# google-research/nerf-from-image

Hardware: AMD Instinct MI355X
Metric: rendered rays/sec (128x128, 64+64 samples) (higher is better)
Workload: dtype f32 (decoder MLP operands split-fp16 hi+lo, 22 bits; strict fp32: config.value_mlp_exact_fp32)

## Files before the change

include/nfi_hip.h:

```cpp
#ifndef NFI_HIP_H
#define NFI_HIP_H

#include <stddef.h>
#include <stdint.h>

#ifdef __cplusplus
extern "C" {
#endif

typedef void* nfi_stream_t;

typedef enum nfi_status {
  NFI_OK = 0,
  NFI_ERR_INVALID_ARGUMENT = -1,
  NFI_ERR_UNSUPPORTED = -2,
  NFI_ERR_WORKSPACE_TOO_SMALL = -3,
  NFI_ERR_LAUNCH = -4
} nfi_status;

enum { NFI_PLANE_CHANNELS = 32, NFI_HIDDEN = 64, NFI_MAX_ATTENTION = 14, NFI_MAX_SAMPLES = 128 };
enum { NFI_MAX_SAMPLES_SINGLE_PASS = 512 };

enum { NFI_TEXEL_F32 = 0, NFI_TEXEL_BF16 = 1, NFI_TEXEL_F16 = 2 };
enum { NFI_TEXELS_PLANAR = 0, NFI_TEXELS_INTERLEAVED = 1 };
// ... 67 lines not shown
  int n_attention;
  const float* attention_values;
  int use_sdf;
  const float* beta;
  const float* alpha;
  float scene_range;
  float* sigma;
  float* rgb;
  float* sdf;
  float* semantics;
  uint8_t* outside;
  const float* ray_features;
  int samples_per_ray;
  int texel_layout;
  int mlp_precision;
} nfi_field_args;
int nfi_field_query_fwd(const nfi_field_args* a, nfi_stream_t stream);
const char* nfi_field_kernel_name(const nfi_field_args* a);

int nfi_bbox_overlay(const float* points, int64_t n_points, float scene_range, float threshold, const float* sigma_in,
                     float* sigma_out, nfi_stream_t stream);

typedef struct nfi_weights_args {
  int64_t n_rays;
  int n_samples;
  const float* sigma;
  const float* ray_directions;
  const float* depth;
  float* weights;
} nfi_weights_args;
int nfi_ray_weights(const nfi_weights_args* a, nfi_stream_t stream);

typedef struct nfi_sample_pdf_args {
  int64_t n_rays;
  int n_bins;
  int n_samples;
  const float* bins;
  const float* weights;
  const float* u;
  int64_t u_row_stride;
  float* samples;
  int64_t* inds;
  float* cdf;
} nfi_sample_pdf_args;
int nfi_sample_pdf(const nfi_sample_pdf_args* a, nfi_stream_t stream);

typedef struct nfi_resample_args {
  int64_t n_rays;
  int n_samples;
  const float* sigma;
  const float* ray_directions;
  const float* depth;
  const float* u;
  int64_t u_row_stride;
  float* fine_depth;
  float* weights;
  float* smooth;
  float* cdf;
  int64_t* inds;
} nfi_resample_args;
int nfi_resample(const nfi_resample_args* a, nfi_stream_t stream);

typedef struct nfi_composite_args {
  int64_t n_rays;
  int n_a;
  int n_b;
  const float* ray_directions;
  const float* depth_a; const float* sigma_a; const float* rgb_a;
  const float* depth_b; const float* sigma_b; const float* rgb_b;
  int n_extra;
  const float* extra_a;
  const float* extra_b;
  int white_background;
  float* rgb_map;
  float* depth_map;
  float* mask;
  float* extra_map;
  float* weights;
  float* depth_sorted;
  int64_t* perm;
} nfi_composite_args;
int nfi_composite_fwd(const nfi_composite_args* a, nfi_stream_t stream);

typedef struct nfi_composite_bwd_args {
  int64_t n_rays;
  int n_a; int n_b;
  const float* ray_directions;
  const float* depth_a; const float* sigma_a; const float* rgb_a;
  const float* depth_b; const float* sigma_b; const float* rgb_b;
  int n_extra; const float* extra_a; const float* extra_b;
  int white_background;
  const float* g_rgb_map;
  const float* g_mask;
  const float* g_extra_map;
  float* g_sigma_a; float* g_rgb_a;
  float* g_sigma_b; float* g_rgb_b;
  float* g_extra_a; float* g_extra_b;
  float* g_ray_directions;
  int list_row_stride;
} nfi_composite_bwd_args;
int nfi_composite_bwd(const nfi_composite_bwd_args* a, nfi_stream_t stream);
int nfi_points_bwd(const float* g_points, const float* depth, int64_t n_rays, int n_samples,
                   float* g_ray_origins, float* g_ray_directions, nfi_stream_t stream);
int nfi_raygen_bwd(const nfi_raygen_args* a, const float* g_ray_origins, const float* g_ray_directions,
                   float* g_cam2world, float* g_focal, nfi_stream_t stream);
int nfi_raygen_bwd_ordered(const nfi_raygen_args* a, const float* g_ray_origins, const float* g_ray_directions,
                           float* g_cam2world, float* g_focal, nfi_stream_t stream);

typedef struct nfi_field_bwd_args {
  int n_scenes;
  int64_t points_per_scene;
  const float* points;
  const void* texels; int plane_res; int texel_dtype;
  const float* decoder_image;
  const float* w1; const float* w2;
  int n_attention; const float* attention_values;
  int use_sdf; const float* beta; const float* alpha;
  float scene_range;
  const float* g_sigma; const float* g_rgb; const float* g_sdf; const float* g_semantics;
  float* g_texels; float* g_points;
  float* g_w1; float* g_b1; float* g_w2; float* g_b2;
  float* g_attention_values; float* g_beta; float* g_alpha;
  void* workspace; size_t workspace_bytes;
  int points_only; int normalize_g_points;
  const float* ray_features; int samples_per_ray; const float* w3;
  float* g_ray_features; float* g_w3; float* g_b3;
  int scatter_mode;
  int texel_layout;
  int rays_per_row;
} nfi_field_bwd_args;
size_t nfi_field_bwd_workspace_bytes(const nfi_field_bwd_args* a);
size_t nfi_decoder_bwd_image_floats(void);
size_t nfi_decoder_bwd_image_floats_viewdir(void);
int nfi_field_query_bwd(const nfi_field_bwd_args* a, nfi_stream_t stream);
const char* nfi_field_bwd_kernel_name(const nfi_field_bwd_args* a);

typedef struct nfi_sdf_gradient_args {
  int n_scenes;
  int64_t points_per_scene;
  const float* points;
  const float* texels; int plane_res;
  float scene_range;
  const float* w1; const float* b1; const float* w2; const float* b2;
  float* sdf; float* gradient;
  const float* g_sdf; const float* g_gradient;
  float* g_texels; float* g_w1; float* g_b1; float* g_w2; float* g_b2;
  int texel_layout;
} nfi_sdf_gradient_args;
int nfi_sdf_gradient_fwd(const nfi_sdf_gradient_args* a, nfi_stream_t stream);
int nfi_sdf_gradient_bwd(const nfi_sdf_gradient_args* a, nfi_stream_t stream);
size_t nfi_sdf_gradient_bwd_ordered_workspace_bytes(const nfi_sdf_gradient_args* a);
int nfi_sdf_gradient_bwd_ordered(const nfi_sdf_gradient_args* a, void* workspace, size_t workspace_bytes, nfi_stream_t stream);

enum { NFI_TUNING_SCANLINE_ORDER = 4, NFI_TUNING_EXACT_FP32_MLP = 8, NFI_TUNING_SINGLE_WORK_COUNTER = 16 };
typedef struct nfi_render_args {
  int n_scenes, height, width;
  int n_samples;
  int fine_sampling;
  int white_background;
  float scene_range;
  int views_per_scene;
  const float* cam2world; const float* focal; const float* bbox; const float* center;
  const void* texels; int plane_res; int texel_dtype;
  const float* decoder_image; int n_attention; const float* attention_values;
  int use_sdf; const float* beta; const float* alpha;
  const float* noise_coarse;
  const float* noise_fine;
  int64_t noise_fine_row_stride;
  float* rgb;
  float* depth;
  float* mask;
  float* semantics;
  float* ray_origins; float* ray_directions; float* near_plane; float* far_plane; uint8_t* hit;
  float* t_coarse; float* sigma_coarse; float* rgb_coarse;
  float* t_fine; float* sigma_fine; float* rgb_fine;
  float* t_sorted; float* weights; int32_t* perm;
  void* workspace; size_t workspace_bytes;
  int skip_missed_rays;
  void* event_start; void* event_stop;
  int tuning;
  void* profile_cycles;
  const float* ray_features;
  float termination_eps;
  int texel_layout;
  void* clock_probe;
  int row_offset; int full_height;
  float* stash_t; float* stash_sigma; float* stash_rgb;
  int rays_ready;
  float* coords;
  float* normals;
} nfi_render_args;
size_t nfi_render_workspace_bytes(int64_t n_rays);
int nfi_render_fwd(const nfi_render_args* a, nfi_stream_t stream);
const char* nfi_render_kernel_name(const nfi_render_args* a);
int nfi_render_setup(const nfi_render_args* a, nfi_stream_t stream);

typedef struct nfi_pnp_args {
  int n_images; int height; int width;
  const float* coords;
  const float* mask;
  float mask_threshold;
  int n_focal; const float* focal_proposals;
  int refine_iterations;
  void* workspace; size_t workspace_bytes;
  float* world2cam;
  float* focal;
  float* error;
} nfi_pnp_args;
size_t nfi_pnp_workspace_bytes(int n_images, int n_focal);
int nfi_pose_pnp(const nfi_pnp_args* a, nfi_stream_t stream);

typedef struct nfi_torgb_args {
  int n_scenes, in_channels, resolution;
  const float* x; const float* styles; const float* weight; const float* bias; const float* previous_image;
  float* texels;
  const float* g_texels;
  float* g_x; float* g_styles; float* g_weight; float* g_bias; float* g_previous_image;
} nfi_torgb_args;
int nfi_torgb_texels_fwd(const nfi_torgb_args* a, nfi_stream_t stream);
int nfi_torgb_texels_bwd(const nfi_torgb_args* a, nfi_stream_t stream);
size_t nfi_torgb_texels_bwd_ordered_workspace_bytes(const nfi_torgb_args* a);
int nfi_torgb_texels_bwd_ordered(const nfi_torgb_args* a, void* workspace, size_t workspace_bytes, nfi_stream_t stream);

typedef struct nfi_warp_args {
  int n_images, channels, height, width;
  const float* image; float* warped;
  const float* g_warped; float* g_image;
  const float* rot; const float* scale; const float* translation;
  int white_background;
} nfi_warp_args;
int nfi_affine_warp_fwd(const nfi_warp_args* a, nfi_stream_t stream);
int nfi_affine_warp_bwd(const nfi_warp_args* a, nfi_stream_t stream);
int nfi_affine_warp_bwd_ordered(const nfi_warp_args* a, nfi_stream_t stream);

typedef struct nfi_metrics_args {
  int n_images;
  const float* pred; const float* target; int64_t elements_per_image;
  const float* mask_pred; const float* mask_real; int64_t elements_per_mask;
  float* psnr; float* iou; int* out_of_range;
} nfi_metrics_args;
int nfi_image_metrics(const nfi_metrics_args* a, nfi_stream_t stream);

typedef struct nfi_viewdir_mapper_args {
  int64_t n_rays;
  const float* viewdir;
  const float *fc0_w, *fc0_b;
  const float *fc1_w, *norm1_w, *norm1_b;
  const float *fc2_w, *norm2_w, *norm2_b;
  const float *fc3_w, *norm3_w, *norm3_b;
  const float *fc4_w, *norm4_w, *norm4_b;
  const float *fc5_w, *fc5_b, *fc6_w, *fc6_b;
  float* feature;
  const float* g_feature;
  float *g_fc0_w, *g_fc0_b;
  float *g_fc1_w, *g_norm1_w, *g_norm1_b;
  float *g_fc2_w, *g_norm2_w, *g_norm2_b;
  float *g_fc3_w, *g_norm3_w, *g_norm3_b;
  float *g_fc4_w, *g_norm4_w, *g_norm4_b;
  float *g_fc5_w, *g_fc5_b, *g_fc6_w, *g_fc6_b;
  float* g_viewdir;
} nfi_viewdir_mapper_args;
int nfi_viewdir_mapper_fwd(const nfi_viewdir_mapper_args* a, nfi_stream_t stream);
int nfi_viewdir_mapper_bwd(const nfi_viewdir_mapper_args* a, nfi_stream_t stream);

#ifdef __cplusplus
}
#endif
#endif
```

nerf_from_image_amd/csrc/nfi_kernels.hip:

```cpp
#include "nfi_device.hpp"
#include "../../include/nfi_hip.h"
#include "nfi_host.hpp"

#include <algorithm>
#include <cstddef>
#include <cstdio>
#include <cstring>

using namespace nfi;

thread_local char nfi_err_buf[256] = "";
extern "C" const char* nfi_last_error(void) { return nfi_err_buf; }
extern "C" int nfi_version(void) { return 102; }


constexpr int kP2tPixels = 256, kP2tPitch = 288;
template <int TEX>
__global__ __launch_bounds__(256) void planes_to_texels_kernel(const float* __restrict__ planes, void* __restrict__ texels,
                                                               int hw) {
  __shared__ __attribute__((aligned(16))) float tile[kC][kP2tPitch];
  const int img = blockIdx.y;
  const int px0 = blockIdx.x * kP2tPixels;
  const float* src = planes + (size_t)img * kC * hw;
  {
// ... 1068 lines not shown
  const int64_t ray = (int64_t)blockIdx.x * 4 + wave;
  if (ray >= a.n_rays) return;
  WaveSlab& slab = slabs[wave];
  const int S = a.n_samples;
  float sigma[2], t[2], u[2], z[2], w[2], sm[2];
  int ind[2];
#pragma unroll
  for (int j = 0; j < 2; ++j) {
    const int e = j * 64 + lane;
    sigma[j] = e < S ? a.sigma[ray * S + e] : 0.0f;
    t[j] = e < S ? a.depth[ray * S + e] : 0.0f;
    u[j] = e < S ? a.u[ray * a.u_row_stride + e] : 0.0f;
  }
  float dn = norm3(a.ray_directions[ray * 3], a.ray_directions[ray * 3 + 1], a.ray_directions[ray * 3 + 2]);
  float Tc[2];
  resample_ray_wide<2>(slab, sigma, t, S, dn, u, lane, z, w, sm, ind, Tc);
#pragma unroll
  for (int j = 0; j < 2; ++j) {
    const int e = j * 64 + lane;
    if (e < S) {
      a.fine_depth[ray * S + e] = z[j];
      if (a.weights) a.weights[ray * S + e] = w[j];
      if (a.smooth) a.smooth[ray * S + e] = sm[j];
      if (a.inds) a.inds[ray * S + e] = ind[j];
    }
    if (a.cdf && e < S - 1) a.cdf[ray * (S - 1) + e] = slab.cdf[e];
  }
}

extern "C" int nfi_resample(const nfi_resample_args* a, nfi_stream_t stream) {
  REQUIRE(a && a->sigma && a->ray_directions && a->depth && a->u && a->fine_depth, "resample: null pointer");
  REQUIRE(a->n_rays > 0 && a->n_samples >= 4 && a->n_samples <= NFI_MAX_SAMPLES, "resample: n_samples must be in [4,128]");
  const dim3 grid((unsigned)((a->n_rays + 3) / 4));
  if (a->n_samples <= 64) hipLaunchKernelGGL(resample_kernel, grid, dim3(256), 0, (hipStream_t)stream, *a);
  else hipLaunchKernelGGL(resample_wide_kernel, grid, dim3(256), 0, (hipStream_t)stream, *a);
  return check_launch("resample");
}

template <int NS>
__global__ __launch_bounds__(256) void composite_kernel(nfi_composite_args a) {
  __shared__ WaveSlabT<64 * NS> slabs[4];
  const int lane = lane_id();
  const int wave = threadIdx.x >> 6;
  const int64_t ray = (int64_t)blockIdx.x * 4 + wave;
  if (ray >= a.n_rays) return;
  auto& slab = slabs[wave];
  const int na = a.n_a, nb = a.n_b, n = na + nb;
  float dep[NS], sig[NS], cr[NS], cg[NS], cb[NS];
  int eidx[NS];
#pragma unroll
  for (int j = 0; j < NS; ++j) {
    int e = j * 64 + lane;
    dep[j] = sig[j] = cr[j] = cg[j] = cb[j] = 0.0f;
    eidx[j] = e;
    if (e < na) {
      size_t i = (size_t)ray * na + e;
      dep[j] = a.depth_a[i]; sig[j] = a.sigma_a[i];
      cr[j] = a.rgb_a[i * 3]; cg[j] = a.rgb_a[i * 3 + 1]; cb[j] = a.rgb_a[i * 3 + 2];
    } else if (e < n) {
      size_t i = (size_t)ray * nb + (e - na);
      dep[j] = a.depth_b[i]; sig[j] = a.sigma_b[i];
      cr[j] = a.rgb_b[i * 3]; cg[j] = a.rgb_b[i * 3 + 1]; cb[j] = a.rgb_b[i * 3 + 2];
    }
  }
  int rank[NS];
  if (nb > 0) {
    merge_scatter<NS>(slab, dep, sig, cr, cg, cb, eidx, n, rank);
  } else {
#pragma unroll
    for (int j = 0; j < NS; ++j) {
      int e = j * 64 + lane;
      rank[j] = e;
      if (e < n) { slab.srt[0][e] = dep[j]; slab.srt[1][e] = sig[j]; slab.srt[2][e] = cr[j]; slab.srt[3][e] = cg[j]; slab.srt[4][e] = cb[j]; }
    }
    wave_lds_fence();
  }
  float dn = norm3(a.ray_directions[ray * 3], a.ray_directions[ray * 3 + 1], a.ray_directions[ray * 3 + 2]);
  float w[NS];
  CompositeOut o = composite_slab<NS>(slab, n, dn, a.white_background, lane, w);
  if (lane == 0) {
    a.rgb_map[ray * 3] = o.r; a.rgb_map[ray * 3 + 1] = o.g; a.rgb_map[ray * 3 + 2] = o.b;
    a.depth_map[ray] = o.depth;
    a.mask[ray] = o.mask;
  }
#pragma unroll
  for (int j = 0; j < NS; ++j) {
    int e = j * 64 + lane;
    if (e < n) {
      if (a.weights) a.weights[(size_t)ray * n + e] = w[j];
      if (a.depth_sorted) a.depth_sorted[(size_t)ray * n + e] = slab.srt[0][e];
      if (a.perm) a.perm[(size_t)ray * n + rank[j]] = e;
    }
  }
  if (a.n_extra > 0 && a.extra_map) {
    wave_lds_fence();
#pragma unroll
    for (int j = 0; j < NS; ++j) {
      int e = j * 64 + lane;
      if (e < n) slab.cdf[e] = w[j];
    }
    wave_lds_fence();
    float we[NS];
#pragma unroll
    for (int j = 0; j < NS; ++j) { int e = j * 64 + lane; we[j] = e < n ? slab.cdf[rank[j]] : 0.0f; }
    for (int c = 0; c < a.n_extra; ++c) {
      float acc = 0.0f;
#pragma unroll
      for (int j = 0; j < NS; ++j) {
        int e = j * 64 + lane;
        if (e < na) acc += we[j] * a.extra_a[((size_t)ray * na + e) * a.n_extra + c];
        else if (e < n) acc += we[j] * a.extra_b[((size_t)ray * nb + (e - na)) * a.n_extra + c];
      }
      acc = wave_sum(acc);
      if (lane == 0) a.extra_map[ray * a.n_extra + c] = acc;
    }
  }
}

extern "C" int nfi_composite_fwd(const nfi_composite_args* a, nfi_stream_t stream) {
  REQUIRE(a && a->ray_directions && a->depth_a && a->sigma_a && a->rgb_a && a->rgb_map && a->depth_map && a->mask,
          "composite: null pointer");
  REQUIRE(a->n_rays > 0 && a->n_a > 0 && a->n_b >= 0 && a->n_a + a->n_b <= NFI_MAX_SAMPLES_SINGLE_PASS,
          "composite: need 1 <= n_a + n_b <= 512");
  REQUIRE(a->n_b == 0 || (a->n_a <= NFI_MAX_SAMPLES && a->n_b <= NFI_MAX_SAMPLES), "composite: merged lists hold at most 128 samples each");
  REQUIRE(a->n_b == 0 || (a->depth_b && a->sigma_b && a->rgb_b), "composite: list b missing");
  REQUIRE(a->n_extra == 0 || (a->extra_a && (a->n_b == 0 || a->extra_b)), "composite: extra attribute missing");
  const dim3 grid((unsigned)((a->n_rays + 3) / 4));
  if (a->n_a + a->n_b <= 128) hipLaunchKernelGGL(composite_kernel<2>, grid, dim3(256), 0, (hipStream_t)stream, *a);
  else if (a->n_a + a->n_b <= 256) hipLaunchKernelGGL(composite_kernel<4>, grid, dim3(256), 0, (hipStream_t)stream, *a);
  else hipLaunchKernelGGL(composite_kernel<8>, grid, dim3(256), 0, (hipStream_t)stream, *a);
  return check_launch("composite_fwd");
}

#include "nfi_backward_rays.inc"
#include "nfi_regulariser.inc"
#include "nfi_neighbours.inc"
#include "nfi_handoff.inc"
#include "nfi_pnp.inc"
#include "nfi_viewdir_mapper.inc"

struct RenderKernelParams {
  int n_scenes, hw, S;
  int fine, white;
  float scene_range;
  const float* ro; const float* rd; const float* near_raw; const float* far_raw; const uint8_t* hit;
  const uint32_t* reduce;
  uint32_t* counter;
  int width;
  int tile_order;
  int xcd_blocks;
  uint32_t* xcd_counter;
  int xcd_block_shift;
  int fetch_batch;
  const void* texels; int res; int layout;
  const float* image; int A; const float* att;
  int use_sdf; const float* beta; const float* alpha;
  const float* noise_c; const float* noise_f; int64_t noise_f_stride;
  float* rgb; float* depth; float* mask;
  float* near_plane; float* far_plane;
  float* t_coarse; float* sigma_coarse; float* rgb_coarse;
  float* t_fine; float* sigma_fine; float* rgb_fine;
  float* t_sorted; float* weights; int32_t* perm;
  int skip_missed;
  unsigned long long* prof;
  const float* xray;
  float term_eps;
  float* semantics;
  float* coords;
  float* normals;
  unsigned long long* clock_probe;
  FastDiv div_scene_rays, div_bps, div_bw;
  int tap_stride;
  int stash;
};

struct ClockProbe {
  unsigned long long c0 = 0, r0 = 0;
  bool on = false;
  __device__ __forceinline__ void start(const RenderKernelParams& k) {
    on = k.clock_probe && blockIdx.x == 0 && threadIdx.x == 0;
    if (on) { c0 = __builtin_readcyclecounter(); r0 = __builtin_amdgcn_s_memrealtime(); }
  }
  __device__ __forceinline__ void stop(const RenderKernelParams& k) const {
    if (on) {
      k.clock_probe[0] = __builtin_readcyclecounter() - c0;
      k.clock_probe[1] = __builtin_amdgcn_s_memrealtime() - r0;
    }
  }
};

__device__ __forceinline__ float uniform_f32(float v) {
  return bits2f((uint32_t)__builtin_amdgcn_readfirstlane((int)f2bits(v)));
}

struct RayInputs {
  float ox, oy, oz, dx, dy, dz, near, far, noise, u;
  uint32_t hit;
};

struct RayQueue {
  const RenderKernelParams& k;
  int lane;
  uint32_t n_rays, xcd, bsh, bw, bps, n_blocks, q_cur, pos_next, pos_end, batch, tiles_x;
  bool dry;
  __device__ __forceinline__ RayQueue(const RenderKernelParams& kk, int l) : k(kk), lane(l) {
    n_rays = (uint32_t)k.n_scenes * (uint32_t)k.hw;
    xcd = k.xcd_blocks ? (__builtin_amdgcn_s_getreg(6164) & 7u) : 0u;
    bsh = (uint32_t)k.xcd_block_shift;
    bw = (uint32_t)k.width >> bsh;
    bps = bw * (((uint32_t)k.hw / (uint32_t)k.width) >> bsh);
    n_blocks = bps * (uint32_t)k.n_scenes;
    q_cur = xcd; pos_next = 0; pos_end = 0; dry = false;
    batch = (uint32_t)k.fetch_batch;
    tiles_x = (uint32_t)k.width >> 3;
  }
  __device__ __forceinline__ uint32_t ray_at(uint32_t q, uint32_t pos) const {
    const uint32_t b = (pos >> (2 * bsh)) * 8u + q;
    const uint32_t in = pos & ((1u << (2 * bsh)) - 1u), scene = fastdiv(b, k.div_bps), bb = b - scene * bps;
    const uint32_t by = fastdiv(bb, k.div_bw), bx = bb - by * bw;
    const uint32_t st = in >> 6, sty = st >> (bsh - 3), stx = st & ((1u << (bsh - 3)) - 1u);
    const uint32_t y = (by << bsh) + (sty << 3) + ((in >> 3) & 7u), x = (bx << bsh) + (stx << 3) + (in & 7u);
    return scene * (uint32_t)k.hw + y * (uint32_t)k.width + x;
  }
  __device__ __forceinline__ uint32_t fetch() {
    if (!k.xcd_blocks) {
      uint32_t p = 0;
      if (lane == 0) p = atomicAdd(k.counter, 1u);
      return (uint32_t)__builtin_amdgcn_readfirstlane((int)p);
    }
    if (pos_next == pos_end && !dry) {
      dry = true;
      for (uint32_t i = 0; i < 8; ++i) {
        uint32_t base = 0;
        if (lane == 0) base = atomicAdd(k.xcd_counter + q_cur * 16, batch);
        base = (uint32_t)__builtin_amdgcn_readfirstlane((int)base);
        if ((base >> (2 * bsh)) * 8u + q_cur < n_blocks) { pos_next = base; pos_end = base + batch; dry = false; break; }
        q_cur = (q_cur + 1) & 7u;
      }
    }
    if (dry) return n_rays;
    return ray_at(q_cur, pos_next++);
  }
  __device__ __forceinline__ bool claimed() const { return pos_next != pos_end; }
  __device__ __forceinline__ uint32_t take() { return ray_at(q_cur, pos_next++); }
  __device__ __forceinline__ uint32_t claim_issue() const {
    uint32_t raw = 0, off = k.xcd_blocks ? q_cur * 16 : 0;
    asm volatile("" : "+v"(off));
    if (k.xcd_blocks && (claimed() || dry)) return raw;
    if (lane == 0) raw = atomicAdd((k.xcd_blocks ? k.xcd_counter : k.counter) + off, k.xcd_blocks ? batch : 1u);
    return raw;
  }
  __device__ __forceinline__ uint32_t claim_finish(uint32_t raw) {
    const uint32_t base = (uint32_t)__builtin_amdgcn_readfirstlane((int)raw);
    if (!k.xcd_blocks) return base;
    if (!claimed() && !dry) {
      if ((base >> (2 * bsh)) * 8u + q_cur < n_blocks) { pos_next = base; pos_end = base + batch; }
      else q_cur = (q_cur + 1) & 7u;
    }
    return fetch();
  }
  __device__ __forceinline__ uint32_t ray_of(uint32_t pos) const {
    if (k.xcd_blocks || !k.tile_order) return pos;
    const uint32_t scene = pos / (uint32_t)k.hw, p = pos - scene * (uint32_t)k.hw;
    const uint32_t tile = p >> 6, in = p & 63u;
    const uint32_t ty = tile / tiles_x, tx = tile - ty * tiles_x;
    return scene * (uint32_t)k.hw + ((ty << 3) + (in >> 3)) * (uint32_t)k.width + (tx << 3) + (in & 7u);
  }
};

constexpr int kRenderPlain = 0, kRenderTaps = 1, kRenderProf = 2, kRenderTerm = 3, kRenderExtra = 4, kRenderNormals = 5;
constexpr int kSemPitch = 2 * 64 + 4;
constexpr int kSemPitchWide = 2 * 128 + 8;
extern __shared__ __attribute__((aligned(16))) float nfi_dyn_lds[];

typedef __attribute__((address_space(3))) float lds_float;

template <int NS, class Slab>
__device__ __forceinline__ void composite_coords(const Slab& slab, const float (&w)[NS], int n, int lane, float ox, float oy,
                                                 float oz, float dx, float dy, float dz, float* out3) {
  float cx = 0.0f, cy = 0.0f, cz = 0.0f;
#pragma unroll
  for (int j = 0; j < NS; ++j) {
    const int e = j * 64 + lane;
    if (e < n) {
      const float t = slab.srt[0][e];
      cx += w[j] * (ox + dx * t); cy += w[j] * (oy + dy * t); cz += w[j] * (oz + dz * t);
    }
  }
  cx = wave_sum(cx); cy = wave_sum(cy); cz = wave_sum(cz);
  if (lane == 0) { out3[0] = cx; out3[1] = cy; out3[2] = cz; }
}


template <int PREC, int kImg>
__device__ __forceinline__ void stage_decoder_image(float* lds, const float* image) {
  if (PREC == 1) {
    for (int i = threadIdx.x; i < kB1F; i += blockDim.x) lds[i] = image[kW1H + i];
    for (int i = kB1F + threadIdx.x; i < kLdsImageFloats; i += blockDim.x) lds[i] = image[i];
  } else {
    for (int i = threadIdx.x; i < kImg; i += blockDim.x) lds[i] = image[i];
  }
  __syncthreads();
}

template <int TEX>
__device__ __forceinline__ void enter_scene(FieldParams& P, const RenderKernelParams& k, float* vf, int scene, int lane) {
  const size_t tb = TEX == 0 ? 128 : 64;
  const char* tex_scene = reinterpret_cast<const char*>(k.texels) + (size_t)scene * 3 * k.res * k.res * tb;
  P.rsrc = __builtin_amdgcn_make_buffer_rsrc(const_cast<char*>(tex_scene), 0, (int)P.scene_bytes, 0x00020000);
  wave_lds_fence();
  {
    int c = lane & 3, row = lane >> 2;
    float v = 0.0f;
    if (k.att && c < 3 && row >= 1 && row <= k.A) v = k.att[((size_t)scene * k.A + (row - 1)) * 3 + c];
    vf[lane] = v;
  }
  wave_lds_fence();
}

__device__ __forceinline__ void store_pixel(const RenderKernelParams& k, uint32_t ray, float r, float g, float b, float depth,
                                            float mask) {
  k.rgb[(size_t)ray * 3] = r; k.rgb[(size_t)ray * 3 + 1] = g; k.rgb[(size_t)ray * 3 + 2] = b;
  k.depth[ray] = depth; k.mask[ray] = mask;
}

__device__ __forceinline__ void store_sample_tap(float* t_out, float* sigma_out, float* rgb_out, size_t i, float t, float sigma,
                                                 float r, float g, float b) {
  if (t_out) t_out[i] = t;
  if (sigma_out) sigma_out[i] = sigma;
  if (rgb_out) { float* q = rgb_out + i * 3; q[0] = r; q[1] = g; q[2] = b; }
}

template <int NS, class Slab>
__device__ __forceinline__ void store_sorted_taps(const RenderKernelParams& k, const Slab& slab, const float (&w)[NS], uint32_t ray,
                                                  int n, int lane) {
#pragma unroll
  for (int j = 0; j < NS; ++j) {
    const int e = j * 64 + lane;
    if (e < n) {
      if (k.weights) k.weights[(size_t)ray * n + e] = w[j];
      if (k.t_sorted) k.t_sorted[(size_t)ray * n + e] = slab.srt[0][e];
    }
  }
}

template <bool NRM>
__device__ __forceinline__ void zero_missed_maps(const RenderKernelParams& k, uint32_t ray, int lane, float bg) {
  if (k.coords && lane < 3) k.coords[(size_t)ray * 3 + lane] = 0.0f;
  if (k.semantics && lane < k.A) k.semantics[(size_t)ray * k.A + lane] = 0.0f;
  if (NRM && lane < 3) k.normals[(size_t)ray * 3 + lane] = bg;
}

__device__ __forceinline__ void zero_stash_row(const RenderKernelParams& k, uint32_t ray, int S, int lane) {
  for (int e = lane; e < S; e += 64) {
    const size_t zs = (size_t)ray * (size_t)k.tap_stride + e;
    k.t_coarse[zs] = 0.0f; k.sigma_coarse[zs] = 0.0f;
    float* q = k.rgb_coarse + zs * 3; q[0] = 0.0f; q[1] = 0.0f; q[2] = 0.0f;
    if (k.fine) {
      k.t_fine[zs] = 0.0f; k.sigma_fine[zs] = 0.0f;
      q = k.rgb_fine + zs * 3; q[0] = 0.0f; q[1] = 0.0f; q[2] = 0.0f;
    }
  }
}

template <bool EXTRA, bool NRM, bool TAPS>
__device__ __forceinline__ void put_missed_ray(const RenderKernelParams& k, uint32_t ray, int S, int lane, float bg) {
  if (lane == 0) store_pixel(k, ray, bg, bg, bg, 0.0f, 0.0f);
  if constexpr (EXTRA) zero_missed_maps<NRM>(k, ray, lane, bg);
  if constexpr (TAPS) {
    if (k.stash) zero_stash_row(k, ray, S, lane);
  }
}

__device__ __forceinline__ uint32_t hit_bytes_scalar(const RenderKernelParams& k, uint32_t ra, uint32_t rb) {
  typedef __attribute__((address_space(4))) const uint32_t const_u32;
  const uintptr_t pa = reinterpret_cast<uintptr_t>(k.hit) + (uint32_t)__builtin_amdgcn_readfirstlane((int)ra),
                  pb = reinterpret_cast<uintptr_t>(k.hit) + (uint32_t)__builtin_amdgcn_readfirstlane((int)rb);
  uint32_t wa = *reinterpret_cast<const_u32*>(pa & ~(uintptr_t)3), wb = *reinterpret_cast<const_u32*>(pb & ~(uintptr_t)3);
  asm volatile("" : "+s"(wa), "+s"(wb));
  return ((wa >> ((uint32_t)(pa & 3) * 8u)) & 0xffu) | (((wb >> ((uint32_t)(pb & 3) * 8u)) & 0xffu) << 8);
}

template <bool EXTRA, bool NRM, bool TAPS, class Load>
__device__ __forceinline__ void skip_miss_run(RayQueue& queue, const RenderKernelParams& k, int S, int lane, float bg,
                                              uint32_t& cur, uint32_t& nxt, Load&& load) {
  put_missed_ray<EXTRA, NRM, TAPS>(k, queue.ray_of(cur), S, lane, bg);
  uint32_t a = nxt;
  while (a < queue.n_rays) {
    const bool two = queue.claimed();
    const uint32_t b = two ? queue.take() : a;
    const uint32_t ra = queue.ray_of(a), rb = queue.ray_of(b);
    const uint32_t hits = hit_bytes_scalar(k, ra, rb);
    uint32_t claim;
    bool ends = true;
    if (hits & 2u) {
      cur = a; load(ra);
      if (two) { nxt = b; return; }
      claim = queue.claim_issue();
    } else if (two && (hits & 0x200u)) {
      put_missed_ray<EXTRA, NRM, TAPS>(k, ra, S, lane, bg);
      cur = b; load(rb);
      claim = queue.claim_issue();
// ... 387 lines not shown
            ws[j] = val[j] ? slab.cdf[rank[j]] : 0.0f;
            ws[2 + j] = (val[j] && k.fine) ? slab.cdf[rank[2 + j]] : 0.0f;
          }
        }
        if constexpr (NRM) {
          const float bgn = k.white ? 1.0f - o.mask : 0.0f;
          float m3[3];
#pragma unroll
          for (int c = 0; c < 3; ++c)
            m3[c] = wave_sum((ws[0] * nrm[0][c] + ws[1] * nrm[1][c]) + (ws[2] * nrm[2][c] + ws[3] * nrm[3][c])) + bgn;
          if (lane == 0) { float* q = k.normals + (size_t)ray * 3; q[0] = m3[0]; q[1] = m3[1]; q[2] = m3[2]; }
        }
        if constexpr (SEMP != 0) {
          if (semT) {
            const lds_u16* sl = (const lds_u16*)semT;
            float mine = 0.0f;
            for (int a = 0; a < k.A; ++a) {
              const lds_u16* row = sl + a * kSemPitchWide + lane;
              const float sa = wave_sum((ws[0] * (float)row[0] + ws[1] * (float)row[64]) + (ws[2] * (float)row[128] + ws[3] * (float)row[192]));
              if (lane == a) mine = sa * (1.0f / 65535.0f);
            }
            const float tot = wave_sum(mine);
            if (tot > 0.0f) mine *= o.mask / tot;
            if (lane < k.A) k.semantics[(size_t)ray * k.A + lane] = mine;
          }
        }
      }
      if constexpr (TAPS) {
        if (lane == 0) {
          if (k.near_plane) k.near_plane[ray] = near;
          if (k.far_plane) k.far_plane[ray] = far;
        }
#pragma unroll
        for (int j = 0; j < 2; ++j) {
          if (val[j]) {
            store_sample_tap(k.t_coarse, k.sigma_coarse, k.rgb_coarse, ts + j * 64 + lane, tc[j], sc[j], rc[j], gc[j], bc[j]);
            if (k.perm) {
              k.perm[(size_t)ray * n + rank[j]] = j * 64 + lane;
              if (k.fine) k.perm[(size_t)ray * n + rank[2 + j]] = S + j * 64 + lane;
            }
          }
        }
        store_sorted_taps<4>(k, slab, w, ray, n, lane);
      }
      wave_lds_fence();
    }
    cur = nxt;
  }
  clock.stop(k);
}

#endif
#ifdef NFI_SINGLE_WIDE
template __global__ void render_fwd_wide_kernel<NFI_SINGLE_KERNEL, true, NFI_SINGLE_MODE, 1, false, NFI_RENDER_OCC>(RenderKernelParams);
#endif
#ifndef NFI_SINGLE_KERNEL
struct __attribute__((aligned(16))) WaveSlabLong {
  float srt[5][NFI_MAX_SAMPLES_SINGLE_PASS];
  float stage[16 * 36];
};

template <int TEX, bool ATT, int PREC, bool VD = false>
__global__ __launch_bounds__(256, NFI_RENDER_OCC) void render_fwd_long_kernel(RenderKernelParams k) {
  constexpr int kImg = VD ? kVdImageFloats : kLdsImageFloats;
  constexpr int NS = NFI_MAX_SAMPLES_SINGLE_PASS / 64;
  __shared__ __attribute__((aligned(16))) float lds[kImg];
  __shared__ __attribute__((aligned(16))) float vfs[4][64];
  __shared__ WaveSlabLong slabs[4];
  ClockProbe clock;
  clock.start(k);
  stage_decoder_image<PREC, kImg>(lds, k.image);
  const int lane = lane_id();
  const int wave = threadIdx.x >> 6;
  WaveSlabLong& slab = slabs[wave];
  float* vf = vfs[wave];
  const int S = k.S;
  const int slots = (S + 63) >> 6;
  const float fill_near = ordered_key_inv(~k.reduce[0]), fill_far = ordered_key_inv(k.reduce[1]);
  const float bg = k.white ? 1.0f : 0.0f;
  const uint32_t n_rays = (uint32_t)k.n_scenes * (uint32_t)k.hw;
  FieldParams P = make_field_params(k.texels, k.res, TEX, k.A, k.use_sdf, k.beta, k.alpha, lds, kImg, k.layout);
  P.vf = vf;
  int cur_scene = -1;
  RayQueue queue(k, lane);
  uint32_t cur = queue.fetch(), nxt = 0;
  while (cur < n_rays) {
    nxt = queue.fetch();
    const uint32_t ray = queue.ray_of(cur);
    const uint32_t hitb = k.hit[ray];
    const size_t ts = (size_t)ray * (size_t)k.tap_stride;
    if (k.skip_missed && !(hitb & 2)) {
      if (lane == 0) store_pixel(k, ray, bg, bg, bg, 0.0f, 0.0f);
      if (k.stash) zero_stash_row(k, ray, S, lane);
    } else {
      const int scene = (int)fastdiv(ray, k.div_scene_rays);
      if (scene != cur_scene) {
        cur_scene = scene;
        enter_scene<TEX>(P, k, vf, scene, lane);
      }
      const size_t r3 = (size_t)ray * 3;
      const float ox = k.ro[r3], oy = k.ro[r3 + 1], oz = k.ro[r3 + 2];
      const float dx = k.rd[r3], dy = k.rd[r3 + 1], dz = k.rd[r3 + 2];
      float near = k.near_raw[ray], far = k.far_raw[ray];
      finish_planes((hitb & 1) != 0, fill_near, fill_far, near, far);
      const float dnorm = norm3(dx, dy, dz);
      const size_t rs = (size_t)ray * S;
#pragma unroll 1
      for (int j = 0; j < slots; ++j) {
        const int e = j * 64 + lane;
        const bool val = e < S;
        const float nz = (k.noise_c && val) ? k.noise_c[rs + e] : 0.0f;
        const float t = val ? stratified_depth(near, far, e, S, nz, k.noise_c != nullptr) : 0.0f;
        SampleOut q = field_wave<TEX, ATT, true, PREC, VD, 0, false, false>(P, k.scene_range, lane, ox + dx * t, oy + dy * t,
                                                                            oz + dz * t, val, nullptr, nullptr, slab.stage,
                                                                            nullptr, nullptr, k.xray, (int)ray);
        if (val) {
          slab.srt[0][e] = t; slab.srt[1][e] = q.sigma; slab.srt[2][e] = q.r; slab.srt[3][e] = q.g; slab.srt[4][e] = q.b;
          store_sample_tap(k.t_coarse, k.sigma_coarse, k.rgb_coarse, ts + e, t, q.sigma, q.r, q.g, q.b);
        }
      }
      wave_lds_fence();
      float w[NS];
      CompositeOut o = composite_slab<NS>(slab, S, dnorm, k.white, lane, w);
      if (lane == 0) {
        store_pixel(k, ray, o.r, o.g, o.b, o.depth, o.mask);
        if (k.near_plane) k.near_plane[ray] = near;
        if (k.far_plane) k.far_plane[ray] = far;
      }
      if (k.weights || k.t_sorted) store_sorted_taps<NS>(k, slab, w, ray, S, lane);
      if (k.perm) {
        for (int e = lane; e < S; e += 64) k.perm[rs + e] = e;
      }
      wave_lds_fence();
    }
    cur = nxt;
  }
  clock.stop(k);
}

struct RenderWorkspaceHeader {
  uint32_t reduce[3];
  uint32_t counter;
  uint32_t pad[12];
  uint32_t xcd_counter[8][16];
};
static_assert(sizeof(RenderWorkspaceHeader) == 64 + 8 * 64 && offsetof(RenderWorkspaceHeader, xcd_counter) == 64,
              "the render workspace header is read from Python and by the kernels' 16-dword counter stride");

static size_t render_workspace_prefix_bytes(int64_t n_rays) {
  size_t n = (size_t)n_rays;
  return sizeof(RenderWorkspaceHeader) + n * 8 * sizeof(float) + ((n + 63) & ~(size_t)63);
}

extern "C" size_t nfi_render_workspace_bytes(int64_t n_rays) {
  return render_workspace_prefix_bytes(n_rays) + kRayBlocks * sizeof(RayPartial);
}

__global__ __launch_bounds__(256) void raygen_finish_kernel(const RayPartial* __restrict__ partial, int n_partials,
                                                            RenderWorkspaceHeader* __restrict__ head) {
  uint32_t kmin = 0u, kmax = 0u, cnt = 0u;
  for (int i = threadIdx.x; i < n_partials; i += blockDim.x) {
    const RayPartial p = partial[i];
    kmin = p.kmin > kmin ? p.kmin : kmin;
    kmax = p.kmax > kmax ? p.kmax : kmax;
    cnt += p.cnt;
  }
  block_reduce_keys(kmin, kmax, cnt);
  uint32_t* cells = reinterpret_cast<uint32_t*>(head);
  for (int i = 3 + threadIdx.x; i < (int)(sizeof(RenderWorkspaceHeader) / sizeof(uint32_t)); i += blockDim.x) cells[i] = 0u;
  if (threadIdx.x == 0) { head->reduce[0] = kmin; head->reduce[1] = kmax; head->reduce[2] = cnt; }
}

struct RenderWorkspace {
  RenderWorkspaceHeader* head; float* ro; float* rd; float* near_raw; float* far_raw; uint8_t* hit; RayPartial* partial; int64_t n;
};

static int render_carve(const nfi_render_args* a, RenderWorkspace& w) {
  REQUIRE(a && a->cam2world && a->workspace, "render: null pointer");
  REQUIRE(a->n_scenes > 0 && a->height > 0 && a->width > 0, "render: bad image shape");
  const int64_t n = (int64_t)a->n_scenes * a->height * a->width;
  if (a->workspace_bytes < nfi_render_workspace_bytes(n)) return fail(NFI_ERR_WORKSPACE_TOO_SMALL, "render: workspace too small");
  w.n = n;
  w.head = reinterpret_cast<RenderWorkspaceHeader*>(a->workspace);
  float* rays = reinterpret_cast<float*>(w.head + 1);
  w.ro = a->ray_origins ? a->ray_origins : rays;
  w.rd = a->ray_directions ? a->ray_directions : rays + 3 * n;
  w.near_raw = rays + 6 * n;
  w.far_raw = rays + 7 * n;
  w.hit = a->hit ? a->hit : reinterpret_cast<uint8_t*>(rays + 8 * n);
  w.partial = reinterpret_cast<RayPartial*>(reinterpret_cast<char*>(a->workspace) + render_workspace_prefix_bytes(n));
  return NFI_OK;
}

static int render_setup(const nfi_render_args* a, const RenderWorkspace& w, hipStream_t s) {
  const int full_h = a->full_height > 0 ? a->full_height : a->height;
  REQUIRE(a->row_offset >= 0 && a->row_offset + a->height <= full_h, "render: row window outside the image");
  CameraParams cam{a->cam2world, a->focal, a->bbox, a->focal ? a->center : nullptr, full_h, a->width, 1, a->height, a->row_offset};
  RaygenOut rout{w.ro, w.rd, w.near_raw, w.far_raw, w.hit, w.partial, a->scene_range};
  const int blocks = (int)std::min<int64_t>((w.n + 255) / 256, kRayBlocks);
  hipLaunchKernelGGL(raygen_kernel, dim3((unsigned)blocks), dim3(256), 0, s, cam, a->n_scenes, rout);
  hipLaunchKernelGGL(raygen_finish_kernel, dim3(1), dim3(256), 0, s, w.partial, blocks, w.head);
  return NFI_OK;
}

extern "C" int nfi_render_setup(const nfi_render_args* a, nfi_stream_t stream) {
  RenderWorkspace w;
  int rc = render_carve(a, w);
  if (rc) return rc;
  rc = render_setup(a, w, (hipStream_t)stream);
  if (rc) return rc;
  return check_launch("render_setup");
}

struct RenderFlags { bool stash, debug_tap, any_tap, strict, term, extra; };

static RenderFlags render_flags(const nfi_render_args* a) {
  RenderFlags f;
  f.stash = a->stash_t || a->stash_sigma || a->stash_rgb;
  f.debug_tap = a->t_coarse || a->sigma_coarse || a->rgb_coarse || a->t_fine || a->sigma_fine || a->rgb_fine ||
                a->t_sorted || a->weights || a->perm || a->near_plane || a->far_plane;
  f.any_tap = f.debug_tap || f.stash;
  f.strict = (a->tuning & NFI_TUNING_EXACT_FP32_MLP) != 0;
  f.term = a->termination_eps > 0.0f;
  f.extra = a->semantics || a->coords || a->normals;
  return f;
}

static int render_check_call(const nfi_render_args* a) {
  REQUIRE(a && a->cam2world && a->rgb && a->depth && a->mask && a->workspace, "render: null pointer");
  REQUIRE(a->n_scenes > 0 && a->height > 0 && a->width > 0, "render: bad image shape");
  REQUIRE(a->views_per_scene >= 0, "render: views_per_scene must not be negative (0 and 1 both mean one view)");
  REQUIRE(a->n_scenes % std::max(a->views_per_scene, 1) == 0, "render: n_scenes (the number of images) must be a multiple of views_per_scene");
  REQUIRE(a->n_samples >= 4 && a->n_samples <= (a->fine_sampling ? NFI_MAX_SAMPLES : NFI_MAX_SAMPLES_SINGLE_PASS),
          "render: n_samples must be in [4,128] per pass with fine sampling, [4,512] for a single pass");
  REQUIRE(a->n_samples <= 64 || !a->profile_cycles, "render: the cycle profile exists for n_samples <= 64 only");
  REQUIRE(a->n_samples <= NFI_MAX_SAMPLES || !(a->semantics || a->coords || a->normals),
          "render: semantics / coords / normals maps exist for n_samples <= 128");
  REQUIRE(!a->fine_sampling || a->noise_fine, "render: fine sampling needs u (noise_fine)");
  REQUIRE(!a->semantics || a->n_attention > 0, "render: composited semantics need attention values (A > 0)");
  return check_field_common(a->texels, a->plane_res, a->texel_dtype, a->decoder_image, a->n_attention,
                            a->attention_values, a->use_sdf, a->beta, a->alpha, a->texel_layout);
}

static int render_check_variant(const nfi_render_args* a, const RenderFlags& f) {
  REQUIRE(!f.stash || (a->stash_t && a->stash_sigma && a->stash_rgb), "render: the training stash needs stash_t, stash_sigma and stash_rgb");
  REQUIRE(!f.stash || !(a->t_coarse || a->sigma_coarse || a->rgb_coarse || a->t_fine || a->sigma_fine || a->rgb_fine),
          "render: the training stash and the per-sample debug taps are mutually exclusive");
  REQUIRE(!a->normals || a->use_sdf, "render: the normals map needs the SDF decoder (use_sdf)");
  REQUIRE(a->termination_eps >= 0.0f && a->termination_eps < 1.0f, "render: termination_eps must be in [0,1)");
  REQUIRE(!f.term || a->fine_sampling, "render: termination_eps acts on the fine pass (fine_sampling)");
  REQUIRE(!f.term || !(f.any_tap || f.extra || a->profile_cycles || a->ray_features || f.strict),
          "render: termination_eps cannot be combined with stage taps, extra maps, the cycle profile, the view-direction decoder or the exact-fp32 MLP");
  REQUIRE(!f.extra || !(f.any_tap || a->profile_cycles || f.strict),
          "render: semantics / coords / normals maps cannot be combined with stage taps, the cycle profile or the exact-fp32 MLP");
  REQUIRE(!(f.extra && a->ray_features) || a->texel_dtype == NFI_TEXEL_F32,
          "render: with the view-direction decoder the semantics / coords / normals maps exist for fp32 texels");
  REQUIRE(!(f.strict || a->profile_cycles) || a->texel_dtype == NFI_TEXEL_F32,
          "render: the exact-fp32 MLP (tuning bit 3) and the cycle profile exist for fp32 texels");
  REQUIRE(!(a->ray_features && a->profile_cycles), "render: no cycle profile with the view-direction decoder");
  return NFI_OK;
}

static RenderKernelParams render_kernel_params(const nfi_render_args* a, const RenderWorkspace& w, const RenderFlags& f) {
  RenderKernelParams k;
  memset(&k, 0, sizeof(k));
  k.n_scenes = a->n_scenes; k.hw = a->height * a->width; k.S = a->n_samples;
  k.fine = a->fine_sampling; k.white = a->white_background; k.scene_range = a->scene_range;
  k.ro = w.ro; k.rd = w.rd; k.near_raw = w.near_raw; k.far_raw = w.far_raw; k.hit = w.hit; k.reduce = w.head->reduce;
  k.texels = a->texels; k.res = a->plane_res; k.layout = a->texel_layout; k.image = a->decoder_image; k.A = a->n_attention; k.att = a->attention_values;
  k.use_sdf = a->use_sdf; k.beta = a->beta; k.alpha = a->alpha;
  k.noise_c = a->noise_coarse; k.noise_f = a->noise_fine; k.noise_f_stride = a->noise_fine_row_stride;
  k.rgb = a->rgb; k.depth = a->depth; k.mask = a->mask;
  k.near_plane = a->near_plane; k.far_plane = a->far_plane;
  k.t_coarse = a->t_coarse; k.sigma_coarse = a->sigma_coarse; k.rgb_coarse = a->rgb_coarse;
  k.t_fine = a->t_fine; k.sigma_fine = a->sigma_fine; k.rgb_fine = a->rgb_fine;
  k.tap_stride = a->n_samples;
  if (f.stash) {
    k.tap_stride = (a->fine_sampling ? 2 : 1) * a->n_samples; k.stash = 1;
    k.t_coarse = a->stash_t; k.sigma_coarse = a->stash_sigma; k.rgb_coarse = a->stash_rgb;
    if (a->fine_sampling) {
      k.t_fine = a->stash_t + a->n_samples;
      k.sigma_fine = a->stash_sigma + a->n_samples;
      k.rgb_fine = a->stash_rgb + 3 * (size_t)a->n_samples;
    }
  }
  k.t_sorted = a->t_sorted; k.weights = a->weights; k.perm = a->perm;
  k.skip_missed = (a->skip_missed_rays && !f.debug_tap) ? 1 : 0;

  k.counter = &w.head->counter;
  k.xcd_counter = &w.head->xcd_counter[0][0];
  k.width = a->width;
  k.fetch_batch = 2;
  const int both = a->width | a->height;
  k.xcd_block_shift = (both & 31) == 0 ? 5 : ((both & 15) == 0 ? 4 : 3);
  const int side = 1 << k.xcd_block_shift;
  k.xcd_blocks = (!(a->tuning & NFI_TUNING_SINGLE_WORK_COUNTER) && (a->width % side == 0) && (a->height % side == 0)) ? 1 : 0;
  const uint32_t bw = (uint32_t)a->width >> k.xcd_block_shift, bh = (uint32_t)a->height >> k.xcd_block_shift;
  k.div_scene_rays = make_fastdiv((uint32_t)k.hw * (uint32_t)std::max(a->views_per_scene, 1));
  k.div_bw = make_fastdiv(bw > 0 ? bw : 1u);
  k.div_bps = make_fastdiv(bw * bh > 0 ? bw * bh : 1u);
  k.tile_order = (!(a->tuning & NFI_TUNING_SCANLINE_ORDER) && (a->width % 8 == 0) && (a->height % 8 == 0)) ? 1 : 0;
  k.prof = (unsigned long long*)a->profile_cycles;
  k.xray = a->ray_features;
  k.clock_probe = reinterpret_cast<unsigned long long*>(a->clock_probe);
  k.term_eps = a->termination_eps;
  k.semantics = a->semantics; k.coords = a->coords; k.normals = a->normals;
  return k;
}

using RenderKernel = void (*)(RenderKernelParams);
struct RenderLaunch {
  RenderKernel kernel;
  const char* name;
  int occ;
  size_t max_lds;
  int (*raise_lds)(size_t, const char*);
};
static constexpr char kFwdFamily[] = "render_fwd_kernel", kWideFamily[] = "render_fwd_wide_kernel", kLongFamily[] = "render_fwd_long_kernel";
template <int TEX, bool ATT, int OCC, int MODE, int PREC, bool VD = false>
static RenderLaunch fwd_launch(size_t max_lds = 0) {
  constexpr auto kernel = &render_fwd_kernel<TEX, ATT, OCC, MODE, PREC, VD>;
  return {kernel, KernelName<kFwdFamily, TEX, ATT, OCC, MODE, PREC, VD>::value.s, OCC, max_lds, &ensure_dynamic_lds<kernel>};
}
template <int TEX, bool ATT, int MODE, int PREC, bool VD = false>
static RenderLaunch wide_launch(size_t max_lds = 0) {
  constexpr auto kernel = &render_fwd_wide_kernel<TEX, ATT, MODE, PREC, VD, NFI_RENDER_OCC>;
  return {kernel, KernelName<kWideFamily, TEX, ATT, MODE, PREC, VD, NFI_RENDER_OCC>::value.s, NFI_RENDER_OCC, max_lds, &ensure_dynamic_lds<kernel>};
}
template <int TEX, bool ATT, int PREC, bool VD = false>
static RenderLaunch long_launch() {
  constexpr auto kernel = &render_fwd_long_kernel<TEX, ATT, PREC, VD>;
  return {kernel, KernelName<kLongFamily, TEX, ATT, PREC, VD>::value.s, NFI_RENDER_OCC, 0, &ensure_dynamic_lds<kernel>};
}

static RenderLaunch select_render_kernel(const nfi_render_args* a, const RenderFlags& f) {
  const bool wide = a->n_samples > 64;
  const bool lng = a->n_samples > NFI_MAX_SAMPLES;
  const bool vd = a->ray_features != nullptr, normals = a->normals != nullptr, prof = a->profile_cycles != nullptr;
  constexpr int OCC = NFI_RENDER_OCC;
  constexpr size_t kSemLdsMax = ((size_t)4 * NFI_MAX_ATTENTION * kSemPitch + kNrmLdsFloats) * sizeof(float);
  constexpr size_t kSemLdsMaxWide = (size_t)4 * NFI_MAX_ATTENTION * kSemPitchWide * sizeof(unsigned short) + kNrmLdsFloats * sizeof(float);
  return dispatch_texel_att(a->texel_dtype, a->n_attention > 0, [&](auto tex, auto att) -> RenderLaunch {
    constexpr int TEX = decltype(tex)::value;
    constexpr bool ATT = decltype(att)::value;
    if (lng) {
      if (vd) return long_launch<TEX, ATT, 0, true>();
      if (f.strict) return long_launch<0, ATT, 0>();
      return long_launch<TEX, ATT, 1>();
    }
    if (vd) {
      if constexpr (TEX == 0) {
        if (normals) return wide ? wide_launch<0, ATT, kRenderNormals, 0, true>(kSemLdsMaxWide)
                                 : fwd_launch<0, ATT, OCC, kRenderNormals, 0, true>(kSemLdsMax);
        if (f.extra) return wide ? wide_launch<0, ATT, kRenderExtra, 0, true>(kSemLdsMaxWide)
                                 : fwd_launch<0, ATT, OCC, kRenderExtra, 0, true>(kSemLdsMax);
      }
      return wide ? wide_launch<TEX, ATT, kRenderTaps, 0, true>()
                  : fwd_launch<TEX, ATT, OCC, kRenderTaps, 0, true>();
    }
    if (wide) {
      if (normals) return wide_launch<TEX, ATT, kRenderNormals, 1>(kSemLdsMaxWide);
      if (f.extra) return wide_launch<TEX, ATT, kRenderExtra, 1>(kSemLdsMaxWide);
      if (f.term) return wide_launch<TEX, ATT, kRenderTerm, 1>();
      if (f.any_tap && f.strict) return wide_launch<0, ATT, kRenderTaps, 0>();
      if (f.any_tap) return wide_launch<TEX, ATT, kRenderTaps, 1>();
      if (f.strict) return wide_launch<0, ATT, kRenderPlain, 0>();
      return wide_launch<TEX, ATT, kRenderPlain, 1>();
    }
    if (normals) return fwd_launch<TEX, ATT, OCC, kRenderNormals, 1>(kSemLdsMax);
    if (f.extra) return fwd_launch<TEX, ATT, OCC, kRenderExtra, 1>(kSemLdsMax);
    if (f.term) return fwd_launch<TEX, ATT, OCC, kRenderTerm, 1>();
    if (prof) return fwd_launch<0, ATT, OCC, kRenderProf, 1>();
    if (f.any_tap && f.strict) return fwd_launch<0, ATT, OCC, kRenderTaps, 0>();
    if (f.any_tap) return fwd_launch<TEX, ATT, OCC, kRenderTaps, 1>();
    if (f.strict) return fwd_launch<0, ATT, OCC, kRenderPlain, 0>();
    if constexpr (TEX != 0) return fwd_launch<TEX, ATT, 3, kRenderPlain, 1>();
    else return fwd_launch<TEX, ATT, OCC, kRenderPlain, 1>();
  });
}

extern "C" const char* nfi_render_kernel_name(const nfi_render_args* a) {
  if (render_check_call(a)) return nullptr;
  const RenderFlags f = render_flags(a);
  if (render_check_variant(a, f)) return nullptr;
  return select_render_kernel(a, f).name;
}

extern "C" int nfi_render_fwd(const nfi_render_args* a, nfi_stream_t stream) {
  int rc = render_check_call(a);
  if (rc) return rc;
  RenderWorkspace w;
  rc = render_carve(a, w);
  if (rc) return rc;
  hipStream_t s = (hipStream_t)stream;
  REQUIRE(!(a->rays_ready && (a->ray_origins || a->ray_directions || a->hit || a->stash_t)),
          "render: rays_ready needs the ray set-up in the workspace (no ray_origins / ray_directions / hit taps, no stash)");
  if (!a->rays_ready) {
    rc = render_setup(a, w, s);
    if (rc) return rc;
  }
  const RenderFlags f = render_flags(a);
  rc = render_check_variant(a, f);
  if (rc) return rc;
  const RenderKernelParams k = render_kernel_params(a, w, f);
  const RenderLaunch launch = select_render_kernel(a, f);
  const size_t lds = (a->semantics ? (size_t)4 * a->n_attention * (a->n_samples > 64 ? kSemPitchWide * sizeof(unsigned short) : kSemPitch * sizeof(float)) : 0) +
                     (a->normals ? (size_t)kNrmLdsFloats * sizeof(float) : 0);
  if (launch.max_lds) {
    rc = launch.raise_lds(launch.max_lds, "render");
    if (rc) return rc;
  }
  const int64_t blocks = std::min<int64_t>((int64_t)256 * launch.occ, (w.n + 3) / 4);
  if (a->event_start) (void)hipEventRecord((hipEvent_t)a->event_start, s);
  hipLaunchKernelGGL(launch.kernel, dim3((unsigned)blocks), dim3(256), lds, s, k);
  if (a->event_stop) (void)hipEventRecord((hipEvent_t)a->event_stop, s);
  return check_launch("render_fwd");
}
#endif
```

Baseline: 153.6 million.

## Rebalance XCD block queues with hit-count-sorted block permutation table

```diff
diff --git a/include/nfi_hip.h b/include/nfi_hip.h
--- a/include/nfi_hip.h
+++ b/include/nfi_hip.h
@@ -243,7 +243,8 @@
 size_t nfi_sdf_gradient_bwd_ordered_workspace_bytes(const nfi_sdf_gradient_args* a);
 int nfi_sdf_gradient_bwd_ordered(const nfi_sdf_gradient_args* a, void* workspace, size_t workspace_bytes, nfi_stream_t stream);
 
-enum { NFI_TUNING_SCANLINE_ORDER = 4, NFI_TUNING_EXACT_FP32_MLP = 8, NFI_TUNING_SINGLE_WORK_COUNTER = 16 };
+enum { NFI_TUNING_SCANLINE_ORDER = 4, NFI_TUNING_EXACT_FP32_MLP = 8, NFI_TUNING_SINGLE_WORK_COUNTER = 16,
+       NFI_TUNING_XCD_BLOCKS_IN_ORDER = 32 };
 typedef struct nfi_render_args {
   int n_scenes, height, width;
   int n_samples;
diff --git a/nerf_from_image_amd/csrc/nfi_kernels.hip b/nerf_from_image_amd/csrc/nfi_kernels.hip
--- a/nerf_from_image_amd/csrc/nfi_kernels.hip
+++ b/nerf_from_image_amd/csrc/nfi_kernels.hip
@@ -1244,6 +1244,7 @@
   uint32_t* xcd_counter;
   int xcd_block_shift;
   int fetch_batch;
+  const uint32_t* block_table;
   const void* texels; int res; int layout;
   const float* image; int A; const float* att;
   int use_sdf; const float* beta; const float* alpha;
@@ -1294,6 +1295,7 @@
   const RenderKernelParams& k;
   int lane;
   uint32_t n_rays, xcd, bsh, bw, bps, n_blocks, q_cur, pos_next, pos_end, batch, tiles_x;
+  uint32_t tab_g, tab_b = 0u, nxt_g = 0xffffffffu, nxt_b = 0u;
   bool dry;
   __device__ __forceinline__ RayQueue(const RenderKernelParams& kk, int l) : k(kk), lane(l) {
     n_rays = (uint32_t)k.n_scenes * (uint32_t)k.hw;
@@ -1303,11 +1305,33 @@
     bps = bw * (((uint32_t)k.hw / (uint32_t)k.width) >> bsh);
     n_blocks = bps * (uint32_t)k.n_scenes;
     q_cur = xcd; pos_next = 0; pos_end = 0; dry = false;
+    tab_g = xcd - 8u;
     batch = (uint32_t)k.fetch_batch;
     tiles_x = (uint32_t)k.width >> 3;
   }
-  __device__ __forceinline__ uint32_t ray_at(uint32_t q, uint32_t pos) const {
-    const uint32_t b = (pos >> (2 * bsh)) * 8u + q;
+  __device__ __forceinline__ uint32_t table_entry(uint32_t g) const {
+    typedef __attribute__((address_space(4))) const uint32_t const_u32;
+    const uint32_t e = (g | 15u) < n_blocks ? g ^ 8u : g;
+    return *reinterpret_cast<const_u32*>(reinterpret_cast<uintptr_t>(k.block_table) + (uintptr_t)e * 4u);
+  }
+  __device__ __forceinline__ void table_prefetch() {
+    if (!k.block_table) return;
+    const uint32_t g = tab_g + 8u;
+    if (g < n_blocks && g != nxt_g) { nxt_g = g; nxt_b = table_entry(g); }
+  }
+  __device__ __forceinline__ void table_pin() {
+    if (k.block_table) asm volatile("" : "+s"(nxt_b));
+  }
+  __device__ __forceinline__ uint32_t block_at(uint32_t g) {
+    if (!k.block_table) return g;
+    if (g != tab_g) {
+      tab_b = g == nxt_g ? nxt_b : table_entry(g);
+      tab_g = g;
+    }
+    return tab_b;
+  }
+  __device__ __forceinline__ uint32_t ray_at(uint32_t q, uint32_t pos) {
+    const uint32_t b = block_at((uint32_t)__builtin_amdgcn_readfirstlane((int)((pos >> (2 * bsh)) * 8u + q)));
     const uint32_t in = pos & ((1u << (2 * bsh)) - 1u), scene = fastdiv(b, k.div_bps), bb = b - scene * bps;
     const uint32_t by = fastdiv(bb, k.div_bw), bx = bb - by * bw;
     const uint32_t st = in >> 6, sty = st >> (bsh - 3), stx = st & ((1u << (bsh - 3)) - 1u);
@@ -1322,9 +1346,11 @@
     }
     if (pos_next == pos_end && !dry) {
       dry = true;
+      table_prefetch();
       for (uint32_t i = 0; i < 8; ++i) {
         uint32_t base = 0;
         if (lane == 0) base = atomicAdd(k.xcd_counter + q_cur * 16, batch);
+        if (i == 0) table_pin();
         base = (uint32_t)__builtin_amdgcn_readfirstlane((int)base);
         if ((base >> (2 * bsh)) * 8u + q_cur < n_blocks) { pos_next = base; pos_end = base + batch; dry = false; break; }
         q_cur = (q_cur + 1) & 7u;
@@ -1335,11 +1361,13 @@
   }
   __device__ __forceinline__ bool claimed() const { return pos_next != pos_end; }
   __device__ __forceinline__ uint32_t take() { return ray_at(q_cur, pos_next++); }
-  __device__ __forceinline__ uint32_t claim_issue() const {
+  __device__ __forceinline__ uint32_t claim_issue() {
     uint32_t raw = 0, off = k.xcd_blocks ? q_cur * 16 : 0;
     asm volatile("" : "+v"(off));
     if (k.xcd_blocks && (claimed() || dry)) return raw;
+    table_prefetch();
     if (lane == 0) raw = atomicAdd((k.xcd_blocks ? k.xcd_counter : k.counter) + off, k.xcd_blocks ? batch : 1u);
+    table_pin();
     return raw;
   }
   __device__ __forceinline__ uint32_t claim_finish(uint32_t raw) {
@@ -2033,12 +2061,69 @@
   return sizeof(RenderWorkspaceHeader) + n * 8 * sizeof(float) + ((n + 63) & ~(size_t)63);
 }
 
+static size_t render_workspace_table_offset(int64_t n_rays) {
+  return render_workspace_prefix_bytes(n_rays) + kRayBlocks * sizeof(RayPartial);
+}
+
 extern "C" size_t nfi_render_workspace_bytes(int64_t n_rays) {
-  return render_workspace_prefix_bytes(n_rays) + kRayBlocks * sizeof(RayPartial);
-}
+  return render_workspace_table_offset(n_rays) + ((size_t)n_rays / 64) * sizeof(uint32_t);
+}
+
+struct BlockGeometry { int shift, ok; uint32_t bw, bh, n_blocks; };
+static BlockGeometry render_block_geometry(const nfi_render_args* a) {
+  BlockGeometry g;
+  const int both = a->width | a->height;
+  g.shift = (both & 31) == 0 ? 5 : ((both & 15) == 0 ? 4 : 3);
+  const int side = 1 << g.shift;
+  g.ok = (a->width % side == 0) && (a->height % side == 0) ? 1 : 0;
+  g.bw = (uint32_t)a->width >> g.shift; g.bh = (uint32_t)a->height >> g.shift;
+  g.n_blocks = g.bw * g.bh * (uint32_t)a->n_scenes;
+  return g;
+}
+
+__device__ __forceinline__ uint32_t count_wide_hits(const uint8_t* p, int bytes) {
+  uint32_t c = 0;
+  if (bytes == 16 && (reinterpret_cast<uintptr_t>(p) & 15) == 0) {
+    const uint4 v = *reinterpret_cast<const uint4*>(p);
+    c = __popc(v.x & 0x02020202u) + __popc(v.y & 0x02020202u) + __popc(v.z & 0x02020202u) + __popc(v.w & 0x02020202u);
+  } else if ((reinterpret_cast<uintptr_t>(p) & 3) == 0) {
+    for (int i = 0; i < bytes; i += 4) c += __popc(*reinterpret_cast<const uint32_t*>(p + i) & 0x02020202u);
+  } else {
+    for (int i = 0; i < bytes; ++i) c += (p[i] >> 1) & 1u;
+  }
+  return c;
+}
+
+struct BlockTableParams { const uint8_t* hit; uint32_t* table; int shift, width, hw; uint32_t bw, bps, n_blocks, groups; };
 
 __global__ __launch_bounds__(256) void raygen_finish_kernel(const RayPartial* __restrict__ partial, int n_partials,
-                                                            RenderWorkspaceHeader* __restrict__ head) {
+                                                            RenderWorkspaceHeader* __restrict__ head, BlockTableParams t) {
+  if (blockIdx.x != 0) {
+    __shared__ uint32_t s_part[256], s_count[16];
+    const uint32_t G = blockIdx.x - 1, i = threadIdx.x >> 4, sub = threadIdx.x & 15u;
+    const uint32_t b = 16u * G + i, scene = b / t.bps, bb = b - scene * t.bps, by = bb / t.bw, bx = bb - by * t.bw;
+    const uint8_t* base = t.hit + (size_t)scene * (size_t)t.hw + (size_t)(by << t.shift) * (size_t)t.width + (bx << t.shift);
+    const int side = 1 << t.shift, cw = side < 16 ? side : 16, per_row = side / cw;
+    uint32_t c = 0;
+    for (int ch = (int)sub; ch < side * per_row; ch += 16)
+      c += count_wide_hits(base + (size_t)(ch / per_row) * (size_t)t.width + (ch % per_row) * cw, cw);
+    s_part[threadIdx.x] = c;
+    __syncthreads();
+    if (threadIdx.x < 16) {
+      uint32_t sum = 0;
+      for (int j = 0; j < 16; ++j) sum += s_part[threadIdx.x * 16 + j];
+      s_count[threadIdx.x] = sum;
+    }
+    __syncthreads();
+    if (threadIdx.x < 16) {
+      const uint32_t me = threadIdx.x, mine = s_count[me];
+      uint32_t r = 0;
+      for (uint32_t j = 0; j < 16; ++j) r += (s_count[j] > mine || (s_count[j] == mine && j < me)) ? 1u : 0u;
+      const uint32_t pair = r < 8 ? r : 15u - r, x = (pair + G) & 7u;
+      t.table[16u * G + (r < 8 ? 0u : 8u) + x] = 16u * G + me;
+    }
+    return;
+  }
   uint32_t kmin = 0u, kmax = 0u, cnt = 0u;
   for (int i = threadIdx.x; i < n_partials; i += blockDim.x) {
     const RayPartial p = partial[i];
@@ -2050,10 +2135,11 @@
   uint32_t* cells = reinterpret_cast<uint32_t*>(head);
   for (int i = 3 + threadIdx.x; i < (int)(sizeof(RenderWorkspaceHeader) / sizeof(uint32_t)); i += blockDim.x) cells[i] = 0u;
   if (threadIdx.x == 0) { head->reduce[0] = kmin; head->reduce[1] = kmax; head->reduce[2] = cnt; }
+  for (uint32_t g = 16u * t.groups + threadIdx.x; g < t.n_blocks; g += blockDim.x) t.table[g] = g;
 }
 
 struct RenderWorkspace {
-  RenderWorkspaceHeader* head; float* ro; float* rd; float* near_raw; float* far_raw; uint8_t* hit; RayPartial* partial; int64_t n;
+  RenderWorkspaceHeader* head; float* ro; float* rd; float* near_raw; float* far_raw; uint8_t* hit; RayPartial* partial; uint32_t* block_table; int64_t n;
 };
 
 static int render_carve(const nfi_render_args* a, RenderWorkspace& w) {
@@ -2070,6 +2156,7 @@
   w.far_raw = rays + 7 * n;
   w.hit = a->hit ? a->hit : reinterpret_cast<uint8_t*>(rays + 8 * n);
   w.partial = reinterpret_cast<RayPartial*>(reinterpret_cast<char*>(a->workspace) + render_workspace_prefix_bytes(n));
+  w.block_table = reinterpret_cast<uint32_t*>(reinterpret_cast<char*>(a->workspace) + render_workspace_table_offset(n));
   return NFI_OK;
 }
 
@@ -2080,7 +2167,10 @@
   RaygenOut rout{w.ro, w.rd, w.near_raw, w.far_raw, w.hit, w.partial, a->scene_range};
   const int blocks = (int)std::min<int64_t>((w.n + 255) / 256, kRayBlocks);
   hipLaunchKernelGGL(raygen_kernel, dim3((unsigned)blocks), dim3(256), 0, s, cam, a->n_scenes, rout);
-  hipLaunchKernelGGL(raygen_finish_kernel, dim3(1), dim3(256), 0, s, w.partial, blocks, w.head);
+  const BlockGeometry g = render_block_geometry(a);
+  const uint32_t n_table = g.ok ? g.n_blocks : (uint32_t)(w.n / 64), groups = g.ok ? g.n_blocks / 16 : 0u;
+  const BlockTableParams t{w.hit, w.block_table, g.shift, a->width, a->height * a->width, g.bw, g.bw * g.bh, n_table, groups};
+  hipLaunchKernelGGL(raygen_finish_kernel, dim3(1 + groups), dim3(256), 0, s, w.partial, blocks, w.head, t);
   return NFI_OK;
 }
 
@@ -2172,11 +2262,11 @@
   k.xcd_counter = &w.head->xcd_counter[0][0];
   k.width = a->width;
   k.fetch_batch = 2;
-  const int both = a->width | a->height;
-  k.xcd_block_shift = (both & 31) == 0 ? 5 : ((both & 15) == 0 ? 4 : 3);
-  const int side = 1 << k.xcd_block_shift;
-  k.xcd_blocks = (!(a->tuning & NFI_TUNING_SINGLE_WORK_COUNTER) && (a->width % side == 0) && (a->height % side == 0)) ? 1 : 0;
-  const uint32_t bw = (uint32_t)a->width >> k.xcd_block_shift, bh = (uint32_t)a->height >> k.xcd_block_shift;
+  const BlockGeometry geo = render_block_geometry(a);
+  k.xcd_block_shift = geo.shift;
+  k.xcd_blocks = (!(a->tuning & NFI_TUNING_SINGLE_WORK_COUNTER) && geo.ok) ? 1 : 0;
+  k.block_table = (k.xcd_blocks && !(a->tuning & NFI_TUNING_XCD_BLOCKS_IN_ORDER)) ? w.block_table : nullptr;
+  const uint32_t bw = geo.bw, bh = geo.bh;
   k.div_scene_rays = make_fastdiv((uint32_t)k.hw * (uint32_t)std::max(a->views_per_scene, 1));
   k.div_bw = make_fastdiv(bw > 0 ? bw : 1u);
   k.div_bps = make_fastdiv(bw * bh > 0 ? bw * bh : 1u);
```

After: 159.2 million, median of 6. +3.6%, better.
